# Goobley/Lightweaver

Measured on AMD Instinct MI355X. Metric: formal_sol_gamma_matrices iters/sec, higher is better.
Workload: dtype f64; 1 GPU; FALC 82-depth H(6)+CaII(6), 5 mu, Bezier3, densified wavelength grid; Nlambda_per_gpu=10240, Nlambda_total=10240, Nspace=82, Nrays=5, active_transitions=25, parallelism=single GPU, sweep=lanes

## Files before the change

include/lwhip.h:

```cpp
#ifndef LWHIP_H
#define LWHIP_H

#include <stddef.h>
#include <stdint.h>

#ifdef __cplusplus
extern "C" {
#endif

#define LWHIP_ABI_VERSION 4


enum { LWHIP_LINE = 0, LWHIP_CONTINUUM = 1 };

enum {
    LWHIP_BC_UNINITIALISED = 0,
    LWHIP_BC_ZERO = 1,
    LWHIP_BC_THERMALISED = 2,
    LWHIP_BC_PERIODIC = 3,
    LWHIP_BC_CALLABLE = 4
};

enum {
    LWHIP_FS_LINEAR_1D = 0,
// ... 347 lines not shown
    int32_t _pad;
    const double* muz;
    const double* vz;
    const double* lowerBc;
    double* I;
    double* depthChi;
    double* depthEta;
    double* depthI;
} lwhip_rays;
int lwhip_compute_rays(lwhip_context* ctx, const lwhip_rays* rays);
int lwhip_batch_compute_rays(lwhip_batch* batch, const lwhip_rays* perColumn);

int lwhip_synchronize(lwhip_context* ctx);

int lwhip_set_zplane_outputs(lwhip_context* ctx, double* zPlaneDown, double* zPlaneUp);

int lwhip_set_stream(lwhip_context* ctx, void* stream);

int lwhip_profile_enable(lwhip_context* ctx, int enable);
int lwhip_sweep_time(lwhip_context* ctx, double* meanMs, int* nLaunches);

int lwhip_algorithmic_bytes(lwhip_context* ctx, double* bytes);
int lwhip_sweep_kind(lwhip_context* ctx);

#ifdef __cplusplus
}
#endif
#endif
```

lightweaver_amd/_abi.py:

```python
import ctypes as C

ABI_VERSION = 4
AXIS_NONE, AXIS_X, AXIS_Z = 0, 1, 2

LINE, CONTINUUM = 0, 1
BC_UNINITIALISED, BC_ZERO, BC_THERMALISED, BC_PERIODIC, BC_CALLABLE = range(5)
FS_LINEAR_1D, FS_BESSER_1D, FS_BEZIER3_1D = range(3)
FS_NAMES = {
    'piecewise_linear_1d': FS_LINEAR_1D,
    'piecewise_besser_1d': FS_BESSER_1D,
    'piecewise_bezier3_1d': FS_BEZIER3_1D,
}
OK, ERR_INVALID, ERR_UNSUPPORTED, ERR_DEVICE, ERR_SINGULAR, ERR_BUSY = range(6)

ATMOS = 1 << 0
BACKGROUND = 1 << 1
PROFILES = 1 << 2
POPS = 1 << 3
NSTAR = 1 << 4
J = 1 << 5
GAMMA = 1 << 6
BC = 1 << 7
RHOPRD = 1 << 8
I = 1 << 9
# ... 197 lines not shown
    ('lwhip_batch_stat_equil', C.c_int, [C.c_void_p]),
    ('lwhip_batch_compute_profiles', C.c_int, [C.c_void_p]),
    ('lwhip_build_intersections', C.c_int, [C.POINTER(lwhip_grid2d), C.POINTER(lwhip_intersection),
                                             C.POINTER(lwhip_intersection), i32p, i32p, C.c_int32,
                                             C.POINTER(lwhip_intersection), C.c_int64, C.POINTER(C.c_int32),
                                             C.POINTER(C.c_int64)]),
    ('lwhip_redistribute_prd', C.c_int, [ctx_p, C.c_int, C.c_double, C.POINTER(lwhip_prd_result)]),
    ('lwhip_prd_pack', C.c_int, [ctx_p, C.POINTER(C.c_void_p), C.POINTER(C.c_size_t)]),
    ('lwhip_prd_partial', C.c_int, [ctx_p]),
    ('lwhip_prd_finalise', C.c_int, [ctx_p, f64p, i32p, f64p, i32p]),
    ('lwhip_ng_configure', C.c_int, [ctx_p, C.c_int, C.c_int, C.c_int]),
    ('lwhip_ng_accelerate', C.c_int, [ctx_p, i32p, f64p, i32p]),
    ('lwhip_time_dep_update', C.c_int, [ctx_p, C.c_int, f64p, C.c_double]),
    ('lwhip_nr_post_update', C.c_int, [ctx_p, C.POINTER(lwhip_nr_args)]),
    ('lwhip_set_depth_range', C.c_int, [ctx_p, C.c_int, C.c_int]),
    ('lwhip_set_djmax_index_mode', C.c_int, [ctx_p, C.c_int]),
    ('lwhip_synchronize', C.c_int, [ctx_p]),
    ('lwhip_set_stream', C.c_int, [ctx_p, C.c_void_p]),
    ('lwhip_set_zplane_outputs', C.c_int, [ctx_p, f64p, f64p]),
    ('lwhip_profile_enable', C.c_int, [ctx_p, C.c_int]),
    ('lwhip_sweep_time', C.c_int, [ctx_p, C.POINTER(C.c_double), C.POINTER(C.c_int)]),
    ('lwhip_algorithmic_bytes', C.c_int, [ctx_p, C.POINTER(C.c_double)]),
    ('lwhip_sweep_kind', C.c_int, [ctx_p]),
    ('lwhip_set_stokes', C.c_int, [ctx_p, C.POINTER(lwhip_stokes)]),
    ('lwhip_compute_polarised_profiles', C.c_int, [ctx_p]),
    ('lwhip_full_stokes_fs', C.c_int, [ctx_p, C.c_int, C.c_int, C.POINTER(lwhip_iter_result)]),
    ('lwhip_batch_compute_polarised_profiles', C.c_int, [C.c_void_p]),
    ('lwhip_batch_full_stokes_fs', C.c_int, [C.c_void_p, C.c_int, C.c_int, C.POINTER(lwhip_iter_result)]),
    ('lwhip_compute_rays', C.c_int, [ctx_p, C.POINTER(lwhip_rays)]),
    ('lwhip_batch_compute_rays', C.c_int, [C.c_void_p, C.POINTER(lwhip_rays)]),
]


def bind(lib):
    for name, restype, argtypes in SYMBOLS:
        fn = getattr(lib, name)
        fn.restype = restype
        fn.argtypes = argtypes
    return lib


def make_nr_args(atomIdxs, stages, backgroundNe, ne, dC=None, nPrev=None, dt=0.0, crsw=1.0):
    import numpy as np
    n = len(atomIdxs)
    idx = np.ascontiguousarray(atomIdxs, dtype=np.int32)

# ... 15 lines not shown
```

lightweaver_amd/context.py:

```python
from __future__ import annotations

import ctypes as C
import os
from dataclasses import dataclass
from typing import Optional

import numpy as np

from . import _abi as abi
from .model import Problem, check_mus

_PKG = os.path.dirname(os.path.abspath(__file__))
LIB_PATH = os.environ.get('LWHIP_LIB') or os.path.join(_PKG, 'liblwhip.so')
_lib = None


class LwHipError(RuntimeError):
    pass


class ExplodingMatrixError(Exception):
    """Singular Gamma in stat_equil (lightweaver.utils.ExplodingMatrixError)."""


# ... 437 lines not shown
            return False
        _check(self.lib, st, 'lwhip_map_host_J')
        return bool(enable)

    def fingerprint_J(self, array=None) -> int:
        import numpy as np
        ptr = (array if array is not None else self.prob.J[self.laStart:self.laEnd]).ctypes.data
        out = C.c_uint64()
        _check(self.lib, self.lib.lwhip_fingerprint_J(self._h, C.c_void_p(ptr), C.byref(out)), 'lwhip_fingerprint_J')
        return out.value

    def profile_enable(self, enable=True):
        _check(self.lib, self.lib.lwhip_profile_enable(self._h, int(enable)), 'lwhip_profile_enable')

    def sweep_time(self):
        ms = C.c_double()
        n = C.c_int()
        _check(self.lib, self.lib.lwhip_sweep_time(self._h, C.byref(ms), C.byref(n)), 'lwhip_sweep_time')
        return ms.value, n.value

    def sweep_kind(self):
        return {0: 'march', 1: 'lanes', 2: '2d'}.get(self.lib.lwhip_sweep_kind(self._h), '?')

    def algorithmic_bytes(self):
        b = C.c_double()
        _check(self.lib, self.lib.lwhip_algorithmic_bytes(self._h, C.byref(b)), 'lwhip_algorithmic_bytes')
        return b.value


def host_fingerprint(array) -> int:
    import numpy as np
    assert array.dtype == np.float64 and array.flags.c_contiguous
    return load_library().lwhip_host_fingerprint(array.ctypes.data_as(abi.f64p), array.size)


def device_count():
    return load_library().lwhip_device_count()
```

lightweaver_amd/csrc/lwhip_api.hip:

```cpp
#include "lwhip_host.h"

namespace
{
thread_local std::string g_lastError;
}

namespace lwhip
{
int fail(int code, const std::string& msg)
{
    g_lastError = msg;
    return code;
}
}

namespace
{
constexpr size_t HB_TAIL = 0, HB_STATUS = 32, HB_ZERO = 40, HB_POPSTATUS = 48, HB_TURNLATE = 56, HB_PRDCTL = 64, HB_CANARY = 96, HB_CHANGE = 128;
constexpr uint64_t HB_CANARY_WORD = 0x6c77686970424c4bull;
constexpr unsigned char HB_DEAD = 0xC5;
struct Quarantine
{
    std::mutex m;
    std::vector<std::pair<unsigned char*, size_t>> blocks;
// ... 702 lines not shown
    DevArena arena;
    H2DBatch h2d;
    auto bail = [&](int code) {
        h2d.close();
        if (c->tablesFrom)
            c->tablesFrom->borrowers--;
        delete c;
        return code;
    };
    if (hipSetDevice(c->device) != hipSuccess)
        return bail(fail(LWHIP_ERR_DEVICE, "hipSetDevice failed"));
    if (opts && opts->stream)
        c->stream = (hipStream_t)opts->stream;
    else
    {
        c->ownStreamShared = like != nullptr && c->batchHint > 1;
        if ((c->ownStreamShared ? stream_acquire_shared(c->device, &c->ownStream) : stream_acquire(c->device, &c->ownStream)) != hipSuccess)
            return bail(fail(LWHIP_ERR_DEVICE, "hipStreamCreate failed"));
        c->stream = c->ownStream;
    }
    if (host_block_init(c) != LWHIP_OK)
        return bail(LWHIP_ERR_DEVICE);
    c->pairRays = dbg_env_int("LWHIP_PAIR_RAYS", 1) != 0;
    c->prdPipeline = dbg_env_int("LWHIP_PRD_PIPELINE", 1) != 0;
    c->prdGeneral = dbg_env_int("LWHIP_PRD_GENERAL", 0) != 0;
    const bool timing = std::getenv("LWHIP_CREATE_TIMING") != nullptr;
    auto now = [] { return std::chrono::steady_clock::now(); };
    auto ms = [](auto a, auto b) { return std::chrono::duration<double, std::milli>(b - a).count(); };
    const auto t0 = now();
    c->structSig = structure_signature(c);
    if (like)
    {
        lwhip_context* owner = like->tablesFrom ? like->tablesFrom : like;
        if (owner->structSig != c->structSig)
            return bail(fail(LWHIP_ERR_INVALID, "lwhip_create_like: the problems differ in structure (sizes, solver, shard, wavelength "
                                                "grid, or a transition's levels / range / coefficients / grid / cross-sections)"));
        c->tablesFrom = owner;
    }
    const bool plainAllocs = poison_on() || sentinel_on() || std::getenv("LWHIP_TRACE_ALLOC") != nullptr;
    if (!plainAllocs)
    {
        if (c->tablesFrom && c->tablesFrom->stateBytes > 0)
        {
            arena.size = c->tablesFrom->stateBytes + (64u << 10);
            if (hipMalloc((void**)&arena.base, arena.size) == hipSuccess && hipMemsetAsync(arena.base, 0, arena.size, c->stream) == hipSuccess)
                c->stateArena = arena.base;
// ... 1064 lines not shown

int lwhip_sweep_time(lwhip_context* c, double* meanMs, int* nLaunches)
{
    if (!c)
        return fail(LWHIP_ERR_INVALID, "null context");
    HIP_TRY(hipSetDevice(c->device));
    int st = collect_profile(c);
    if (st != LWHIP_OK)
        return st;
    if (meanMs)
        *meanMs = c->sweepCount ? c->sweepMs / c->sweepCount : 0.0;
    if (nLaunches)
        *nLaunches = c->sweepCount;
    return LWHIP_OK;
}

int lwhip_sweep_kind(lwhip_context* c)
{
    if (!c)
        return -1;
    return c->is2d ? 2 : c->laneSweep ? 1 : 0;
}

int lwhip_algorithmic_bytes(lwhip_context* c, double* bytes)
{
    if (!c || !bytes)
        return fail(LWHIP_ERR_INVALID, "null argument");
    const double Ns = c->Ns, Nla = c->Nla, Nmu = c->Nrays;
    double sumLineLa = 0.0, gam = 0.0, lev = 0.0;
    for (auto& h : c->trans)
        if (h.t.type == LWHIP_LINE)
            sumLineLa += h.NredLoc - h.NblueLoc;
    for (auto& a : c->atoms)
    {
        lev += a.Nlevel;
        if (!a.detailed)
            gam += 2.0 * a.Nlevel * a.Nlevel;
    }
    double b = 8.0 * Ns * (2.0 * Nmu * sumLineLa + 3.0 * Nla + 2.0 * Nla);
    b += 8.0 * Nla * Nmu * c->Nx;
    b += 8.0 * Ns * (gam + lev);
    b += 8.0 * Ns * 2.0 * c->Ntrans;
    b += 8.0 * Ns * (lev + 3.0 + Nmu);
    *bytes = b;
    return LWHIP_OK;
}
// ... 2 lines not shown
```

lightweaver_amd/csrc/lwhip_batch.hip:

```cpp
#include "lwhip_host.h"


static int batch_compute_profiles(lwhip_batch* b, bool all)
{
    std::vector<VoigtLineArgs> list;
    std::vector<lwhip_context*> todo;
    for (lwhip_context* c : b->ctxs)
    {
        if (!(all || c->profilesStale))
            continue;
        const int st = voigt_line_list(c, list);
        if (st != LWHIP_OK)
            return st;
        todo.push_back(c);
    }
    if (todo.empty())
        return LWHIP_OK;
    lwhip_context* c0 = b->ctxs[0];
    if (!list.empty())
    {
        if (b->voigtList.n < list.size())
        {
            HIP_TRY(hipStreamSynchronize(c0->stream));
            HIP_TRY(b->voigtList.alloc(c0->mem, list.size()));
// ... 184 lines not shown
        if (stp != LWHIP_OK)
            return stp;
    }
    for (int i = 0; i < n; ++i)
    {
        lwhip_context* c = b->ctxs[i];
        if (c->partialPending || c->prdPending)
            return fail(LWHIP_ERR_INVALID, "batch iteration while a split iteration of a column is pending");
        c->prefillCrsw = crsw;
        c->dJPrdClean = false;
        c->prefillPending = c->gammaTot > 0 && c->Cmat.p != nullptr;
        b->aHost[i] = make_apply_args(c);
        c->prefillPending = false;
    }
    if (!b->aValid || b->aCrsw != crsw)
    {
        HIP_TRY(hipMemcpyAsync(b->aList.p, b->aHost.data(), (size_t)n * sizeof(ApplyArgs), hipMemcpyHostToDevice, c0->stream));
        b->aValid = true;
        b->aCrsw = crsw;
    }
    TileDyn dyn = make_dyn(c0, false, lambdaIterate);
    for (int q = 0; q < n && dyn.phiSym; ++q)
        dyn.phiSym = b->ctxs[q]->phiSym ? 1 : 0;
    const bool fuse = c0->tileFuse;
    if (!c0->laneSweep)
        HIP_TRY(launch_tile_pre(c0->dtargs.p, c0->htargs, c0->nTiles, b->apList.p, n, c0->stream));
    if (c0->laneSweep)
        HIP_TRY(launch_lane_sweep(c0->dtargs.p, c0->htargs, dyn, c0->prob.formalSolver, true, c0->nTileChunks, c0->tileWaves, b->apList.p, n,
                                  c0->stream));
    else
    {
        HIP_TRY(launch_tile_sweep(c0->dtargs.p, c0->htargs, dyn, c0->prob.formalSolver, c0->tileCap, true, fuse, c0->nTileChunks,
                                  c0->tileWaves, b->apList.p, n, c0->stream));
        if (!fuse)
            HIP_TRY(launch_tile_post(c0->dtargs.p, c0->htargs, dyn, c0->nPostChunks, b->apList.p, n, c0->stream));
    }
    {
        ReduceArgs r0 = make_reduce_args(c0);
        r0.zeroParts = 1;
        HIP_TRY(launch_reduce_sum(r0, c0->stream, b->rList.p, n));
    }
    if (c0->Natom > 0)
        HIP_TRY(launch_apply(b->aHost[0], c0->stream, b->aList.p, n));
    if (results)
    {
        HIP_TRY(hipMemcpyAsync(b->tailPinned.host, b->tail.p, (size_t)2 * n * sizeof(double), hipMemcpyDeviceToHost, c0->stream));
        HIP_TRY(hipStreamSynchronize(c0->stream));
        for (int i = 0; i < n; ++i)
        {
            results[i].updatedJ = 1;
            results[i].dJMax = b->tailPinned.as<double>()[2 * i];
            results[i].dJMaxIdx = (int32_t)b->tailPinned.as<double>()[2 * i + 1];
// ... 40 lines not shown
```

lightweaver_amd/csrc/lwhip_host.h:

```cpp
#pragma once
#include "lwhip_internal.h"
#include "../../include/lwhip.h"

#include <hip/hip_runtime.h>

#include <algorithm>
#include <array>
#include <atomic>
#include <cmath>
#include <cstdio>
#include <cstdlib>
#include <chrono>
#include <cstring>
#include <functional>
#include <map>
#include <memory>
#include <mutex>
#include <string>
#include <type_traits>
#include <vector>

namespace lwhip
{
int fail(int code, const std::string& msg);
// ... 367 lines not shown
    bool prdPending = false;
    bool prdFused = false;
    std::vector<std::unique_ptr<DevBuf<double>>> gII;
    std::vector<char> gIIValid;
    DevBuf<NrAtom> nrAtoms, statEqAtoms;
    DevBuf<NgAtom> ngAtoms;
    DevBuf<double> ngHistory;
    std::vector<NgAtom> ngAtomsHost;
    int ngOrder = 0, ngPeriod = 0, ngDelay = 0, ngCount = 0;
    bool ngConfigured = false;
    int statEqKey = -2;
    int32_t* statusHost = nullptr;
    int32_t* statusDev = nullptr;
    double* changeHost = nullptr;
    double* changeDev = nullptr;
    size_t changeCount = 0;
    DevBuf<int32_t> transType;
    DevBuf<int32_t> contLa;
    DevBuf<int32_t> prdChangeIdx;
    PinnedBlock prdPinned;
    DevBuf<int32_t> prdCtl;
    bool phiSym = false, vlosZero = false;
    bool pairRays = true, prdPipeline = true, prdGeneral = false;
    PinnedBlock prdPinnedPipe;
    int prdPipeIter = 0;
    double prdPipeTol = 0.0;
    DevBuf<DevTrans> dtrans;
    DevBuf<DevLaHeader> laHdr;
    DevBuf<DevSlot> slots;
    DevBuf<DevProgram> progs;
    DevBuf<DevProgRow> progRows;
    DevBuf<DevProgEnt> progEnts;
    DevBuf<ContArgs> dargs;
    ContArgs hargs{};
    bool atomicParts = false;
    bool red8Clean = false;
    int* zeroCheck = nullptr;
    int* zeroCheckDev = nullptr;
    DevBuf<int32_t> atomTrOffD, atomNlevel, atomDetailed, transLi, transLj;
    DevBuf<int64_t> atomGammaOff;
    DevBuf<double> red, red8, dJ;
    std::vector<double> gatherHost;
    DevBuf<int32_t> status;
    StokesState stokes;
    RaysState* rays = nullptr;

// ... 140 lines not shown
```

lightweaver_amd/csrc/lwhip_internal.h:

```cpp
#pragma once
#include <vector>
#include <hip/hip_runtime.h>
#include <stdint.h>

#include "../../include/lwhip.h"

namespace lwhip
{
constexpr double CLight = 2.99792458E+08;
constexpr double HPlanck = 6.6260755E-34;
constexpr double HC = HPlanck * CLight;
constexpr double KBoltzmann = 1.380658E-23;
constexpr double Pi = 3.14159265358979323846264338327950288;
constexpr double NM_TO_M = 1.0E-09;
constexpr double HC_K = HC / (KBoltzmann * NM_TO_M);
constexpr double HC_4PI = 0.25 * HC / Pi;
constexpr double PI4_HC = 1.0 / HC_4PI;
constexpr double PI4_H = 4.0 * Pi / HPlanck;
constexpr double TWO_HC_NM3 = 2.0 * HC / (NM_TO_M * NM_TO_M * NM_TO_M);

struct DevTrans
{
    int32_t type;
    int32_t atom;
// ... 230 lines not shown
    const int64_t* hJOff;
    const lwhip_j_coeff* hJCoef;
    double* JRest;
    const DevLaneWg* laneWg;
    const DevLaneTile* laneTiles;
    const DevLaneRay* laneRays;
    const DevLaneFin* laneFin;
    const double* laneFinPar;
    const double* bcPlanck;
    const uint8_t* laneFeedG;
    double* momS;
    int32_t momA, _padM;
    int32_t* turnLate;
    double* detSlab;
    double* lsDbg;
};
struct TileDyn
{
    int32_t nPass;
    int32_t lambdaIterate;
    int32_t prdOnly;
    int32_t stopIter;
    const int32_t* stopCtl;
    int32_t phiSym, _padS;
};
struct RetileArgs
{
    int32_t Ns, Nmu, L, nTiles;
    const DevTile* tiles;
    const DevTileSlot* tslots;
    const DevTrans* trans;
    const double* phi;
    double* phiT;
};
size_t raymarch_lds_bytes(const TileArgs& a, int waves, bool fuse);
hipError_t launch_tile_pre(const TileArgs* devArgs, const TileArgs& hostArgs, int nTilesLaunch, const TileArgs* const* apList,
                           int nBatch, hipStream_t stream);
hipError_t launch_tile_sweep(const TileArgs* devArgs, const TileArgs& hostArgs, const TileDyn& dyn, int solver, int cap,
                             bool rates, bool fuse, int nChunks, int waves, const TileArgs* const* apList, int nBatch,
                             hipStream_t stream);
hipError_t launch_tile_post(const TileArgs* devArgs, const TileArgs& hostArgs, const TileDyn& dyn, int nPostChunks,
                            const TileArgs* const* apList, int nBatch, hipStream_t stream);
bool lane_sweep_supported(int Ns, int Nrays, int solver, int* D, int* LR, int* R);
size_t lane_sweep_lds_bytes(const TileArgs& a, int waves);
hipError_t launch_lane_sweep(const TileArgs* devArgs, const TileArgs& hostArgs, const TileDyn& dyn, int solver, bool rates,
                             int nChunks, int waves, const TileArgs* const* apList, int nBatch, hipStream_t stream);
void dbg_scratch_poison(hipStream_t stream);
hipError_t launch_det_reduce(const double* slab, const int32_t* off, const int32_t* ent, double* part, int Ns, int Ntrans,
                             hipStream_t stream);
size_t det_reduce_scratch_doubles(int Ns, int Ntrans);
hipError_t launch_retile(const RetileArgs& a, hipStream_t stream);
hipError_t launch_retile_list(const RetileArgs* devList, const RetileArgs* hostList, int n, hipStream_t stream);

#ifndef LWHIP_REDUCE_SPLIT_N
#define LWHIP_REDUCE_SPLIT_N 4
#endif
enum { LWHIP_REDUCE_SPLIT = LWHIP_REDUCE_SPLIT_N };
enum { LWHIP_DET_SEG = 32 };
struct ReduceArgs
{
    int32_t Ns, Ntrans;
    double* red8;
    double* red;
    const double* dJ;
    int32_t Nla, idxOffset, world, rank;
    double* batchTail;
    int32_t zeroParts;
// ... 312 lines not shown
```

lightweaver_amd/csrc/lwhip_lanesweep.hip:

```cpp
#include "lwhip_device.h"
#include <atomic>
#include <cstdlib>
#include "../../include/lwhip.h"

#include <algorithm>
#include <type_traits>

namespace lwhip
{
namespace
{
typedef unsigned int ls_u2 __attribute__((ext_vector_type(2)));
typedef unsigned int ls_u4 __attribute__((ext_vector_type(4)));

DEVINL __amdgpu_buffer_rsrc_t ls_rsrc(const void* p, unsigned long long bytes)
{
    const unsigned n = bytes > 0xfffffff0ull ? 0xfffffff0u : (unsigned)bytes;
    return __builtin_amdgcn_make_buffer_rsrc((void*)p, 0, (int)n, 0x00020000);
}
template <int N> DEVINL void ls_ld(__amdgpu_buffer_rsrc_t r, unsigned voff, unsigned soff, double (&x)[N])
{
#pragma unroll
    for (int q = 0; q + 1 < N; q += 2)
    {
// ... 31 lines not shown
    const int lo = __builtin_amdgcn_update_dpp(0, (int)(unsigned)vv, CTRL, 0xf, 0xf, true);
    const int hi = __builtin_amdgcn_update_dpp(0, (int)(unsigned)(vv >> 32), CTRL, 0xf, 0xf, true);
    return __longlong_as_double(((unsigned long long)(unsigned)hi << 32) | (unsigned)lo);
}
DEVINL double ls_bperm(double v, int srcLane)
{
    const unsigned long long vv = __double_as_longlong(v);
    const int lo = __builtin_amdgcn_ds_bpermute(srcLane << 2, (int)(unsigned)vv);
    const int hi = __builtin_amdgcn_ds_bpermute(srcLane << 2, (int)(unsigned)(vv >> 32));
    return __longlong_as_double(((unsigned long long)(unsigned)hi << 32) | (unsigned)lo);
}
template <bool UP> DEVINL void ls_scan(double& E, double& B, const int lane, const int LR)
{
#pragma unroll
    for (int s = 1; s < 64; s <<= 1)
    {
        if (s == 32 && LR <= 32)
            break;
        const int src = UP ? lane + s : lane - s;
        const double Ep = ls_bperm(E, src), Bp = ls_bperm(B, src);
        B = fma(E, Bp, B);
        E = E * Ep;
    }
}
DEVINL double ls_rcp(double x)
{
    double r = __builtin_amdgcn_rcp(x);
    const double e = fma(-x, r, 1.0);
    return fma(r, e, r);
}
enum { LS_EXP_TAB = 32 };
DEVINL void ls_exp_table_init(double* tab, int t)
{
    if (t < LS_EXP_TAB)
        tab[t] = exp2((double)t * (1.0 / LS_EXP_TAB));
}
DEVINL double ls_exp_neg(double x, const double* tab)
{
    double k0 = 46.166241308446828384, k1 = -2.16608493865351192653e-02, k2 = -5.96317165397058656257e-12;
    double c6 = 1.0 / 720.0, c5 = 1.0 / 120.0, c4 = 1.0 / 24.0, c3 = 1.0 / 6.0;
    asm volatile("" : "+s"(k0), "+s"(k1), "+s"(k2), "+s"(c6), "+s"(c5), "+s"(c4), "+s"(c3));
    const double n = rint(x * k0);
    double r = fma(n, k1, x);
    r = fma(n, k2, r);
    const int ni = (int)n;
    const double T = tab[ni & (LS_EXP_TAB - 1)];
// ... 745 lines not shown
            LS_T(tp2);
            LS_TACC(tmB, tp1, tp2);
#pragma unroll
            for (int i = 0; i < D; ++i)
            {
                const double Su = SRC(i - 1), S0 = S[i];
                const double xi = x[i];
                const double x2 = xi * xi, x3 = x2 * xi;
                const double exr = ls_exp_neg(-fmin(xi, 64.0), c.sExp);
                const double ex = (xi > 30.0) ? 0.0 : exr;
                const double r3 = (rx[i] * rx[i]) * rx[i];
                const bool small = xi < 5e-2;
                auto pick = [&](double g, double t) {
                    LS_KEEP(g);
                    LS_KEEP(t);
                    double r = small ? t : g;
                    LS_KEEP(r);
                    return r;
                };
                const double xq = 0.25 * xi, q = 0.05 * x2, t3 = x3 * (1.0 / 120.0);
                const double al = pick((6.0 - ex * (6.0 + 6.0 * xi + 3.0 * x2 + x3)) * r3, xq - 4.0 * q + 10.0 * t3);
                const double be = pick((6.0 * ex - 6.0 + 6.0 * xi - 3.0 * x2 + x3) * r3, xq - q + t3);
                const double ga = pick(3.0 * (2.0 * xi - 6.0 + ex * (6.0 + 4.0 * xi + x2)) * r3, xq - 3.0 * q + 6.0 * t3);
                const double de = pick(3.0 * (6.0 - 4.0 * xi + x2 - 2.0 * ex * (3.0 + xi)) * r3, xq - 2.0 * q + 3.0 * t3);
                const double edt = pick(ex, 1.0 - xi + 0.5 * x2 - 20.0 * t3);
                const double x_3 = xi * (1.0 / 3.0);
                const double dSu = i == 0 ? dSP : dS[i > 0 ? i - 1 : 0];
                const double Cuw = Su + x_3 * dSu;
                const double C0 = S0 - x_3 * dS[i];
                double e1 = edt, b1 = al * Su + be * S0 + ga * Cuw + de * C0, ps = be + de;
                LS_KEEP(b1);
                LS_KEEP(ps);
                if (__builtin_amdgcn_ballot_w64(is_last(i)) != 0)
                {
                    double w0 = 1.0 - exr, w1 = (1.0 - exr) - xi * exr;
                    if (xi < 5.0E-4)
                    {
                        w0 = xi * (1.0 - 0.5 * xi);
                        w1 = (xi * xi) * (0.5 - xi * (1.0 / 3.0));
                    }
                    else if (xi > 50.0)
                        w0 = w1 = 1.0;
                    const double rL = ls_rcp(xi);
                    const double dSL = (S0 - Su) * rL;
                    const bool lst = is_last(i);
                    e1 = lst ? 1.0 - w0 : e1;
                    b1 = lst ? w0 * S0 - w1 * dSL : b1;
                    ps = lst ? w0 - w1 * rL : ps;
// ... 467 lines not shown
            static_assert(D % 2 == 0, "the block's rate integrals are formed in halves");
            if (!MOM)
            {
                rates_half(std::integral_constant<int, 0>{});
                LS_PHASE();
                rates_half(std::integral_constant<int, D / 2>{});
            }
        }
        LS_PHASE();
        LS_T(tp5);
        LS_TACC(tmA, tp0, tp1);
        LS_TACC(tmS, tp3, tp4);
        LS_TACC(tmD, tp4, tp5);
#ifdef LS_TIMING
        tmC += tp3 - tp1 - (tmB - tmBprev);
        tmBprev = tmB;
#endif
#undef MI
#undef IV
#undef CHI
#undef SRC
    };

    const int nRun = NRUN;
    for (run = 0; run < nRun; ++run)
    {
    const bool pairMode = PAIRABLE && dyn.phiSym != 0 && dyn.nPass == 2 && q0 == 0 && q1 == 2 * Nmu;
    if (!pairMode)
        prefetch_first();
    if constexpr (CONT)
        cont_unit(0);
#ifdef LS_ABL_NO_RAYS
    if (dyn.nPass == 77)
#else
    if (dyn.nPass == 2)
#endif
    {
        if (pairMode)
        {
            if constexpr (PAIRABLE)
            {
                for (int mu = 0; mu < Nmu; ++mu)
                {
                    cont_unit(mu);
                    pass(std::false_type{}, std::true_type{}, mu, 0u);
                    pass(std::true_type{}, std::true_type{}, mu, 0u);
                }
            }
        }
        else
        {
            for (int mu = q0 >> 1; 2 * mu < q1; ++mu)
            {
                if (2 * mu >= q0)
                    pass(std::false_type{}, std::false_type{}, mu, (unsigned)(mu * 2 + 1) * Ns8);
                if (2 * mu + 1 < q1)
                    pass(std::true_type{}, std::false_type{}, mu, (unsigned)(mu * 2 + 2) * Ns8);
            }
        }
    }
    else
// ... 1676 lines not shown
    *LR = lr;
    *R = std::min(64 / lr, (int)LS_MAX_R);
    return true;
}

size_t det_reduce_scratch_doubles(int Ns, int Ntrans) { return (size_t)std::max(Ntrans, 1) * DET_SEG * 4 * Ns; }

hipError_t launch_det_reduce(const double* slab, const int32_t* off, const int32_t* ent, double* part, int Ns, int Ntrans,
                             hipStream_t stream)
{
    if (Ntrans <= 0)
        return hipSuccess;
    LWHIP_LAUNCH(det_reduce_kernel, dim3((4 * Ns + 255) / 256, Ntrans, DET_SEG), dim3(256), 0, stream, slab, off, ent, part, Ns);
    return hipGetLastError();
}

size_t lane_sweep_lds_bytes(const TileArgs& a, int waves)
{
    return sizeof(double) * ((size_t)a.maxCT * 4 * a.laneLRD + (size_t)waves * LS_MAX_R * 5 + LS_EXP_TAB + (size_t)waves * 3 * 64 * a.laneD
                             + (size_t)waves * std::min(a.maxC, (int)LWHIP_POST_MAXC) * a.L * 3)
           + a.depBytes + (a.detSlab ? ((size_t)a.maxCT * a.laneD * sizeof(int) + 7) / 8 * 8 : 0);
}

#ifndef LS_ISA_ONLY
hipError_t launch_lane_sweep(const TileArgs* devArgs, const TileArgs& a, const TileDyn& dyn, int solver, bool rates, int nChunks,
                             int waves, const TileArgs* const* apList, int nBatch, hipStream_t stream)
{
    if (nChunks <= 0)
        return hipSuccess;
    if (waves < 1 || waves > LS_MAX_WAVES || a.laneD != 4)
        return hipErrorInvalidValue;
    if (solver == LWHIP_FS_LINEAR_1D)
        return rates ? launch_ls_t<LWHIP_FS_LINEAR_1D, 4, 3>(devArgs, a, dyn, nChunks, waves, apList, nBatch, stream)
                     : launch_ls_t<LWHIP_FS_LINEAR_1D, 4, 2>(devArgs, a, dyn, nChunks, waves, apList, nBatch, stream);
    if (solver == LWHIP_FS_BESSER_1D)
        return rates ? launch_ls_t<LWHIP_FS_BESSER_1D, 4, 3>(devArgs, a, dyn, nChunks, waves, apList, nBatch, stream)
                     : launch_ls_t<LWHIP_FS_BESSER_1D, 4, 2>(devArgs, a, dyn, nChunks, waves, apList, nBatch, stream);
    if (solver != LWHIP_FS_BEZIER3_1D)
        return hipErrorInvalidValue;
    const bool hprd = a.hRho != nullptr || a.hJOff != nullptr;
    if (rates)
        return hprd ? launch_ls_t<LWHIP_FS_BEZIER3_1D, 4, 3>(devArgs, a, dyn, nChunks, waves, apList, nBatch, stream)
                    : launch_ls_t<LWHIP_FS_BEZIER3_1D, 4, 1>(devArgs, a, dyn, nChunks, waves, apList, nBatch, stream);
    return hprd ? launch_ls_t<LWHIP_FS_BEZIER3_1D, 4, 2>(devArgs, a, dyn, nChunks, waves, apList, nBatch, stream)
                : launch_ls_t<LWHIP_FS_BEZIER3_1D, 4, 0>(devArgs, a, dyn, nChunks, waves, apList, nBatch, stream);
}
// ... 3 lines not shown
```

lightweaver_amd/csrc/lwhip_state.hip:

```cpp
#include "lwhip_host.h"

namespace lwhip
{
bool poison_on()
{
    static const bool poison = debug_knobs_on() && std::getenv("LWHIP_POISON") != nullptr;
    return poison;
}
bool sentinel_on()
{
    static const bool on = debug_knobs_on() && std::getenv("LWHIP_PAD_SENTINEL") != nullptr && *std::getenv("LWHIP_PAD_SENTINEL");
    return on;
}
static bool sentinel_for(int seq)
{
    if (!sentinel_on())
        return false;
    static int lo = 0, hi = -1;
    static bool parsed = false;
    if (!parsed)
    {
        const char* v = std::getenv("LWHIP_PAD_SENTINEL");
        if (v[0] == 'a')
        {
// ... 455 lines not shown
    r.tslots = c->tslots.p;
    r.trans = c->dtrans.p;
    r.phi = c->phi.p;
    r.phiT = c->phiT.p;
    return true;
}

int retile_profiles(lwhip_context* c)
{
    RetileArgs r;
    if (retile_args(c, r))
        HIP_TRY(launch_retile(r, c->stream));
    return LWHIP_OK;
}

TileDyn make_dyn(lwhip_context* c, bool upOnly, int lambdaIterate)
{
    TileDyn d{};
    d.nPass = upOnly ? 1 : 2;
    d.lambdaIterate = lambdaIterate;
    d.stopIter = 0;
    d.stopCtl = nullptr;
    d.phiSym = (c && c->phiSym && c->pairRays) ? 1 : 0;
    return d;
}

hipError_t run_sweep(lwhip_context* c, const TileDyn& dyn, bool rates, hipEvent_t e0, hipEvent_t e1)
{
    TileDyn td = dyn;
    const bool tprd = dyn.prdOnly != 0;
    if (tprd && c->nTileChunksPrd == 0)
        return hipSuccess;
    if (!tprd)
        c->dJPrdClean = false;
    const TileArgs* da = tprd ? c->dtargsPrd.p : c->dtargs.p;
    const TileArgs& ha = tprd ? c->htargsPrd : c->htargs;
    const bool fuse = c->tileFuse && rates;
    if (rates && c->hprd && c->JRest.p)
    {
        hipError_t ez = hipMemsetAsync(c->JRest.p, 0, c->JRest.n * sizeof(double), c->stream);
        if (ez != hipSuccess)
            return ez;
    }
    if (rates && c->zeroCheckDev)
    {
        hipError_t ec = launch_check_zero(c->red8.p, c->red8.n, c->zeroCheckDev, c->stream);
        if (ec != hipSuccess)
            return ec;
    }
    hipError_t e = c->laneSweep ? hipSuccess : launch_tile_pre(da, ha, tprd ? c->nTilesPrd : c->nTiles, nullptr, 0, c->stream);
    if (e != hipSuccess)
        return e;
    if (e0)
        (void)hipEventRecord(e0, c->stream);
    if (c->laneSweep)
        e = launch_lane_sweep(da, ha, td, c->prob.formalSolver, rates, tprd ? c->nTileChunksPrd : c->nTileChunks, c->tileWaves, nullptr, 0,
                              c->stream);
    else
        e = launch_tile_sweep(da, ha, td, c->prob.formalSolver, c->tileCap, rates, fuse, tprd ? c->nTileChunksPrd : c->nTileChunks,
                              (fuse && ha.depthSplit > 1) ? 2 * ha.depthSplit : c->tileWaves, nullptr, 0, c->stream);
    if (e1)
        (void)hipEventRecord(e1, c->stream);
    if (e == hipSuccess && rates && c->laneSweep && c->deterministic)
        e = launch_det_reduce(c->detSlab.p, tprd ? c->detOffPrd.p : c->detOff.p, tprd ? c->detEntPrd.p : c->detEnt.p, c->detPart.p, c->Ns,
                              c->Ntrans, c->stream);
    if (e != hipSuccess || !rates || fuse || c->laneSweep)
        return e;
    return launch_tile_post(da, ha, td, tprd ? c->nPostChunksPrd : c->nPostChunks, nullptr, 0, c->stream);
}

int flush_prefill(lwhip_context* c)
{
    if (c->prefillPending && c->gammaTot > 0)
        HIP_TRY(launch_prefill(c->Gamma.p, c->Cmat.p, c->prefillCrsw, (size_t)c->gammaTot, c->stream));
    c->prefillPending = false;
    return LWHIP_OK;
}

int verify_zero_check(lwhip_context* c)
{
// ... 455 lines not shown
```

lightweaver_amd/csrc/lwhip_tables.hip:

```cpp
#include "lwhip_host.h"

namespace lwhip
{
int validate(const lwhip_problem* p, std::string& why)
{
    if (!p)
    {
        why = "null problem";
        return LWHIP_ERR_INVALID;
    }
    if (p->abiVersion != LWHIP_ABI_VERSION)
    {
        why = "ABI version mismatch";
        return LWHIP_ERR_INVALID;
    }
    if (p->Nspace < 3 || p->Nrays < 1 || p->Nlambda < 1 || p->Natom < 0)
    {
        why = "need Nspace >= 3, Nrays >= 1, Nlambda >= 1";
        return LWHIP_ERR_INVALID;
    }
    if (p->grid2d)
    {
        const lwhip_grid2d& g = *p->grid2d;
        if (g.Nx < 2 || g.Nz < 2 || g.Nx > 1024 || g.Nx * g.Nz != p->Nspace || g.Nrays != p->Nrays)
// ... 1451 lines not shown
            auto wg_records = [&](const std::vector<int32_t>& chTile, const std::vector<int32_t>* order, const std::vector<int32_t>* split,
                                  int launchSplit) {
                const int nch = (int)chTile.size() - 1;
                std::vector<DevLaneWg> w(std::max(nch, 1));
                for (int b = 0; b < nch; ++b)
                {
                    const int ch = order ? (*order)[b] : b;
                    const int S = split ? (*split)[ch] : launchSplit;
                    w[b] = DevLaneWg{ ch, S > 1 ? S : 1, chTile[ch], chTile[ch + 1] };
                }
                return w;
            };
            std::vector<int32_t> orderHost;
            if (c->chunkOrderOn)
            {
                orderHost.resize(c->chunkOrder.n);
                if (c->mem.batch)
                    HIP_TRY(c->mem.batch->flush());
                HIP_TRY(hipMemcpyAsync(orderHost.data(), c->chunkOrder.p, orderHost.size() * sizeof(int32_t), hipMemcpyDeviceToHost, c->stream));
                HIP_TRY(hipStreamSynchronize(c->stream));
            }
            auto wgs = wg_records(chunkTile, c->chunkOrderOn ? &orderHost : nullptr, c->chunkSplitOn ? &laneChunkSplit : nullptr, c->laneSplit);
            HIP_TRY(c->laneWg.upload_or_borrow(c->mem, wgs, like ? &like->laneWg : nullptr));
            std::vector<int32_t> genOf(std::max<size_t>(tiles.size(), 1), -1);
            std::vector<uint8_t> feedG;
            c->nGenTiles = 0;
            auto feed_byte = [&](const DevSlot& cs, const DevTileSlot& us, bool isThisMixed) -> uint8_t {
                uint32_t b = 0;
                if ((cs.flags & 1) && (us.flags & 1))
                {
                    b |= cs.atom == us.atom ? 1u : 0u;
                    b |= cs.gi == us.gi ? 2u : 0u;
                    b |= cs.gj == us.gi ? 4u : 0u;
                    b |= cs.gi == us.gj ? 8u : 0u;
                    b |= cs.gj == us.gj ? 16u : 0u;
                    b |= cs.gj == us.gi ? 32u : 0u;
                    b |= cs.gj == us.gj ? 64u : 0u;
                }
                if (isThisMixed)
                    b |= 128u;
                return (uint8_t)b;
            };
            for (size_t t = 0; t < tiles.size(); ++t)
            {
                const DevTile& td = tiles[t];
                const bool fastKind = (td.nLine == 0 && td.nMixed == 0) || (td.nLine == 1 && td.nMixed <= 1) || (td.nLine == 2 && td.nMixed == 0);
// ... 154 lines not shown
```

Before: 7712 iters/s.

## Share Bezier3 coefficients between paired up/down rays in lane sweep

Adds a pair_pass in the lane sweep that computes the Bezier3 interpolation coefficients once per depth interval and uses them for both the downward and upward ray of a given mu. The two direction scans then run together in one interleaved prefix scan. This removes duplicated exp and polynomial coefficient work for continuum tiles and phi-symmetric line tiles. It enables this by default through an env flag and adds a debug counter for how many tasks take the path. It also increases register pressure from holding both directions' arrays at once, and disables FMA contraction in two places to keep results matching.

```diff
diff --git a/include/lwhip.h b/include/lwhip.h
--- a/include/lwhip.h
+++ b/include/lwhip.h
@@ -393,6 +393,7 @@
 
 int lwhip_algorithmic_bytes(lwhip_context* ctx, double* bytes);
 int lwhip_sweep_kind(lwhip_context* ctx);
+long lwhip_debug_pair_coef_tasks(lwhip_context* ctx);
 
 #ifdef __cplusplus
 }
diff --git a/lightweaver_amd/_abi.py b/lightweaver_amd/_abi.py
--- a/lightweaver_amd/_abi.py
+++ b/lightweaver_amd/_abi.py
@@ -243,6 +243,7 @@
     ('lwhip_sweep_time', C.c_int, [ctx_p, C.POINTER(C.c_double), C.POINTER(C.c_int)]),
     ('lwhip_algorithmic_bytes', C.c_int, [ctx_p, C.POINTER(C.c_double)]),
     ('lwhip_sweep_kind', C.c_int, [ctx_p]),
+    ('lwhip_debug_pair_coef_tasks', C.c_long, [ctx_p]),
     ('lwhip_set_stokes', C.c_int, [ctx_p, C.POINTER(lwhip_stokes)]),
     ('lwhip_compute_polarised_profiles', C.c_int, [ctx_p]),
     ('lwhip_full_stokes_fs', C.c_int, [ctx_p, C.c_int, C.c_int, C.POINTER(lwhip_iter_result)]),
diff --git a/lightweaver_amd/context.py b/lightweaver_amd/context.py
--- a/lightweaver_amd/context.py
+++ b/lightweaver_amd/context.py
@@ -483,6 +483,9 @@
     def sweep_kind(self):
         return {0: 'march', 1: 'lanes', 2: '2d'}.get(self.lib.lwhip_sweep_kind(self._h), '?')
 
+    def pair_coef_tasks(self):
+        return int(self.lib.lwhip_debug_pair_coef_tasks(self._h))
+
     def algorithmic_bytes(self):
         b = C.c_double()
         _check(self.lib, self.lib.lwhip_algorithmic_bytes(self._h, C.byref(b)), 'lwhip_algorithmic_bytes')
diff --git a/lightweaver_amd/csrc/lwhip_api.hip b/lightweaver_amd/csrc/lwhip_api.hip
--- a/lightweaver_amd/csrc/lwhip_api.hip
+++ b/lightweaver_amd/csrc/lwhip_api.hip
@@ -748,6 +748,7 @@
     if (host_block_init(c) != LWHIP_OK)
         return bail(LWHIP_ERR_DEVICE);
     c->pairRays = dbg_env_int("LWHIP_PAIR_RAYS", 1) != 0;
+    c->pairCoefs = dbg_env_int("LWHIP_PAIR_COEFS", 1) != 0;
     c->prdPipeline = dbg_env_int("LWHIP_PRD_PIPELINE", 1) != 0;
     c->prdGeneral = dbg_env_int("LWHIP_PRD_GENERAL", 0) != 0;
     const bool timing = std::getenv("LWHIP_CREATE_TIMING") != nullptr;
@@ -1858,6 +1859,8 @@
     return c->is2d ? 2 : c->laneSweep ? 1 : 0;
 }
 
+long lwhip_debug_pair_coef_tasks(lwhip_context* c) { return c ? c->pairCoefTasks : 0; }
+
 int lwhip_algorithmic_bytes(lwhip_context* c, double* bytes)
 {
     if (!c || !bytes)
diff --git a/lightweaver_amd/csrc/lwhip_batch.hip b/lightweaver_amd/csrc/lwhip_batch.hip
--- a/lightweaver_amd/csrc/lwhip_batch.hip
+++ b/lightweaver_amd/csrc/lwhip_batch.hip
@@ -230,12 +230,19 @@
     TileDyn dyn = make_dyn(c0, false, lambdaIterate);
     for (int q = 0; q < n && dyn.phiSym; ++q)
         dyn.phiSym = b->ctxs[q]->phiSym ? 1 : 0;
+    for (int q = 0; q < n && dyn.pairCoefs; ++q)
+        dyn.pairCoefs = b->ctxs[q]->pairCoefs ? 1 : 0;
     const bool fuse = c0->tileFuse;
     if (!c0->laneSweep)
         HIP_TRY(launch_tile_pre(c0->dtargs.p, c0->htargs, c0->nTiles, b->apList.p, n, c0->stream));
     if (c0->laneSweep)
+    {
         HIP_TRY(launch_lane_sweep(c0->dtargs.p, c0->htargs, dyn, c0->prob.formalSolver, true, c0->nTileChunks, c0->tileWaves, b->apList.p, n,
                                   c0->stream));
+        for (int q = 0; q < n; ++q)
+            b->ctxs[q]->pairCoefTasks =
+                lane_sweep_pairs_coefs(c0->htargs, dyn, c0->prob.formalSolver) ? c0->pairTasksCont + (dyn.phiSym ? c0->pairTasksLine : 0) : 0;
+    }
     else
     {
         HIP_TRY(launch_tile_sweep(c0->dtargs.p, c0->htargs, dyn, c0->prob.formalSolver, c0->tileCap, true, fuse, c0->nTileChunks,
diff --git a/lightweaver_amd/csrc/lwhip_host.h b/lightweaver_amd/csrc/lwhip_host.h
--- a/lightweaver_amd/csrc/lwhip_host.h
+++ b/lightweaver_amd/csrc/lwhip_host.h
@@ -413,6 +413,9 @@
     DevBuf<int32_t> prdCtl;
     bool phiSym = false, vlosZero = false;
     bool pairRays = true, prdPipeline = true, prdGeneral = false;
+    bool pairCoefs = true;
+    long pairCoefTasks = 0;
+    long pairTasksCont = 0, pairTasksLine = 0;
     PinnedBlock prdPinnedPipe;
     int prdPipeIter = 0;
     double prdPipeTol = 0.0;
diff --git a/lightweaver_amd/csrc/lwhip_internal.h b/lightweaver_amd/csrc/lwhip_internal.h
--- a/lightweaver_amd/csrc/lwhip_internal.h
+++ b/lightweaver_amd/csrc/lwhip_internal.h
@@ -276,7 +276,8 @@
     int32_t prdOnly;
     int32_t stopIter;
     const int32_t* stopCtl;
-    int32_t phiSym, _padS;
+    int32_t phiSym;
+    int32_t pairCoefs;
 };
 struct RetileArgs
 {
@@ -297,6 +298,7 @@
                             const TileArgs* const* apList, int nBatch, hipStream_t stream);
 bool lane_sweep_supported(int Ns, int Nrays, int solver, int* D, int* LR, int* R);
 size_t lane_sweep_lds_bytes(const TileArgs& a, int waves);
+bool lane_sweep_pairs_coefs(const TileArgs& hostArgs, const TileDyn& dyn, int solver);
 hipError_t launch_lane_sweep(const TileArgs* devArgs, const TileArgs& hostArgs, const TileDyn& dyn, int solver, bool rates,
                              int nChunks, int waves, const TileArgs* const* apList, int nBatch, hipStream_t stream);
 void dbg_scratch_poison(hipStream_t stream);
diff --git a/lightweaver_amd/csrc/lwhip_lanesweep.hip b/lightweaver_amd/csrc/lwhip_lanesweep.hip
--- a/lightweaver_amd/csrc/lwhip_lanesweep.hip
+++ b/lightweaver_amd/csrc/lwhip_lanesweep.hip
@@ -77,6 +77,31 @@
         B = fma(E, Bp, B);
         E = E * Ep;
     }
+}
+DEVINL void ls_scan_pair(double& Ed, double& Bd, double& Eu, double& Bu, const int lane, const int LR)
+{
+#pragma unroll
+    for (int s = 1; s < 64; s <<= 1)
+    {
+        if (s == 32 && LR <= 32)
+            break;
+        const double Epd = ls_bperm(Ed, lane - s), Bpd = ls_bperm(Bd, lane - s);
+        const double Epu = ls_bperm(Eu, lane + s), Bpu = ls_bperm(Bu, lane + s);
+        Bd = fma(Ed, Bpd, Bd);
+        Ed = Ed * Epd;
+        Bu = fma(Eu, Bpu, Bu);
+        Eu = Eu * Epu;
+    }
+}
+DEVINL double ls_add_nc(double c, double x)
+{
+#pragma clang fp contract(off)
+    return c + x;
+}
+DEVINL double ls_sub_nc(double c, double x)
+{
+#pragma clang fp contract(off)
+    return c - x;
 }
 DEVINL double ls_rcp(double x)
 {
@@ -868,8 +893,8 @@
                 const double al = pick((6.0 - ex * (6.0 + 6.0 * xi + 3.0 * x2 + x3)) * r3, xq - 4.0 * q + 10.0 * t3);
                 const double be = pick((6.0 * ex - 6.0 + 6.0 * xi - 3.0 * x2 + x3) * r3, xq - q + t3);
                 const double ga = pick(3.0 * (2.0 * xi - 6.0 + ex * (6.0 + 4.0 * xi + x2)) * r3, xq - 3.0 * q + 6.0 * t3);
-                const double de = pick(3.0 * (6.0 - 4.0 * xi + x2 - 2.0 * ex * (3.0 + xi)) * r3, xq - 2.0 * q + 3.0 * t3);
-                const double edt = pick(ex, 1.0 - xi + 0.5 * x2 - 20.0 * t3);
+                const double de = pick(3.0 * (6.0 - 4.0 * xi + x2 - 2.0 * ex * ls_add_nc(3.0, xi)) * r3, xq - 2.0 * q + 3.0 * t3);
+                const double edt = pick(ex, ls_sub_nc(1.0, xi) + 0.5 * x2 - 20.0 * t3);
                 const double x_3 = xi * (1.0 / 3.0);
                 const double dSu = i == 0 ? dSP : dS[i > 0 ? i - 1 : 0];
                 const double Cuw = Su + x_3 * dSu;
@@ -1383,6 +1408,270 @@
 #undef SRC
     };
 
+#ifdef LS_NO_PAIR_COEFS
+    constexpr bool PAIRCOEF = false;
+#else
+    constexpr bool PAIRCOEF = CONT || PAIRABLE;
+#endif
+    auto pair_pass = [&](const int mu) {
+        LS_T(tp0);
+        const double muz = CTAB(double, a.muz)[mu];
+        const double zmu = CTAB(double, a.muz)[Nmu + mu];
+        const double hw = act ? 0.5 * CTAB(double, a.wmu)[mu] : 0.0;
+        int pBot = c.pBot, blk = c.blk, nV = c.nV;
+        LS_KEEPI(pBot);
+        LS_KEEPI(blk);
+        LS_KEEPI(nV);
+        auto dhK = [&](const int q) { return ((const double*)(sDep + c.vK + c.oG))[q]; };
+        if (storeDepth && act)
+        {
+            const size_t o = ((size_t)(la * Nmu + mu) * 2) * Ns + k0;
+#pragma unroll
+            for (int p = 0; p < D; ++p)
+                if (p < c.nV)
+                {
+                    double eC = (c.sRow3 + c.lane * D)[64 * D + p];
+                    if constexpr (PAIRABLE)
+                        eC = fma(cer[0][p], hPhi[p], eC);
+                    GD(a.depthChi)[o + p] = hChi[p];
+                    GD(a.depthEta)[o + p] = eC;
+                    GD(a.depthChi)[o + Ns + p] = hChi[p];
+                    GD(a.depthEta)[o + Ns + p] = eC;
+                }
+        }
+        LS_PHASE();
+        LS_T(tp1);
+        auto chi_at = [&](const int i) {
+            const double* r3 = c.sRow3 + c.lane * D;
+            asm volatile("" : "+v"(r3));
+            double cC = r3[i];
+            if constexpr (PAIRABLE)
+                cC = fma(cxr[0][i], hPhi[i], cC);
+            return cC;
+        };
+        auto chiK = [&](int i) {
+            return i < 0 ? ls_shift1<true>(chi_at(D - 1)) : i >= D ? ls_shift1<false>(chi_at(0)) : chi_at(i < 0 ? 0 : i >= D ? D - 1 : i);
+        };
+        auto srcK = [&](int i) { return i < 0 ? hSLo : i >= D ? hSHi : hS[i < 0 ? 0 : i >= D ? D - 1 : i]; };
+        auto dsK = [&](int i) { return i < 0 ? hDSLo : i >= D ? hDSHi : hDS[i < 0 ? 0 : i >= D ? D - 1 : i]; };
+        struct XCoef
+        {
+            double al, be, ga, de, edt, x_3;
+        };
+        auto x_coefs = [&](const double xi, const double rxi) -> XCoef {
+            const double x2 = xi * xi, x3 = x2 * xi;
+            const double exr = ls_exp_neg(-fmin(xi, 64.0), c.sExp);
+            const double ex = (xi > 30.0) ? 0.0 : exr;
+            const double r3 = (rxi * rxi) * rxi;
+            const bool small = xi < 5e-2;
+            auto pick = [&](double g, double t) {
+                LS_KEEP(g);
+                LS_KEEP(t);
+                double r = small ? t : g;
+                LS_KEEP(r);
+                return r;
+            };
+            const double xq = 0.25 * xi, q = 0.05 * x2, t3 = x3 * (1.0 / 120.0);
+            XCoef k;
+            k.al = pick((6.0 - ex * (6.0 + 6.0 * xi + 3.0 * x2 + x3)) * r3, xq - 4.0 * q + 10.0 * t3);
+            k.be = pick((6.0 * ex - 6.0 + 6.0 * xi - 3.0 * x2 + x3) * r3, xq - q + t3);
+            k.ga = pick(3.0 * (2.0 * xi - 6.0 + ex * (6.0 + 4.0 * xi + x2)) * r3, xq - 3.0 * q + 6.0 * t3);
+            k.de = pick(3.0 * (6.0 - 4.0 * xi + x2 - 2.0 * ex * ls_add_nc(3.0, xi)) * r3, xq - 2.0 * q + 3.0 * t3);
+            k.edt = pick(ex, ls_sub_nc(1.0, xi) + 0.5 * x2 - 20.0 * t3);
+            k.x_3 = xi * (1.0 / 3.0);
+            return k;
+        };
+        auto form_map = [&](auto upTag, const int p, const XCoef& k, double& eo, double& bo, double& po) {
+            constexpr bool UP = decltype(upTag)::value;
+            const int pu = UP ? p + 1 : p - 1, pd = UP ? p - 1 : p + 1;
+            const int bcType = UP ? a.lowerBc : a.upperBc;
+            auto is_first = [&]() { return UP ? p == pBot : (p == 0 && blk == 0); };
+            auto is_last = [&]() { return UP ? (p == 0 && blk == 0) : p == pBot; };
+            auto is_ok = [&]() { return p < nV; };
+            const double Su = srcK(pu), S0 = hS[p];
+            const double dSu = UP ? -(dsK(pu) * muz) : dsK(pu) * muz;
+            const double dS0 = UP ? -(hDS[p] * muz) : hDS[p] * muz;
+            const double Cuw = Su + k.x_3 * dSu;
+            const double C0 = S0 - k.x_3 * dS0;
+            double e1 = k.edt, b1 = k.al * Su + k.be * S0 + k.ga * Cuw + k.de * C0, ps = k.be + k.de;
+            LS_KEEP(b1);
+            LS_KEEP(ps);
+            if (__builtin_amdgcn_ballot_w64(is_last()) != 0)
+            {
+                const bool lst = is_last();
+                const double dtL = ((0.5 * zmu) * (chiK(p) + chiK(pu))) * dhK(UP ? p + 1 : p);
+                const double xi = lst ? dtL : 1.0;
+                const double exr = ls_exp_neg(-fmin(xi, 64.0), c.sExp);
+                double w0 = 1.0 - exr, w1 = (1.0 - exr) - xi * exr;
+                if (xi < 5.0E-4)
+                {
+                    w0 = xi * (1.0 - 0.5 * xi);
+                    w1 = (xi * xi) * (0.5 - xi * (1.0 / 3.0));
+                }
+                else if (xi > 50.0)
+                    w0 = w1 = 1.0;
+                const double rL = ls_rcp(xi);
+                const double dSL = (S0 - Su) * rL;
+                e1 = lst ? 1.0 - w0 : e1;
+                b1 = lst ? w0 * S0 - w1 * dSL : b1;
+                ps = lst ? w0 - w1 * rL : ps;
+            }
+            if (__builtin_amdgcn_ballot_w64(is_first()) != 0)
+            {
+                double Ib = 0.0;
+                if (bcType == LWHIP_BC_THERMALISED)
+                {
+                    const double dtb = ((0.5 * zmu) * (chiK(p) + chiK(pd))) * dhK(UP ? p : p + 1);
+                    const double rdtb = ls_rcp(dtb);
+                    const double* sb = c.sB + min(c.rRaw, LS_MAX_R - 1) * 4 + (UP ? 2 : 0);
+                    const double B0 = sb[0], B1 = sb[1];
+                    Ib = UP ? B1 - (B0 - B1) * rdtb : B0 - (B1 - B0) * rdtb;
+                }
+                else if (bcType == LWHIP_BC_CALLABLE)
+                {
+                    const int mi = UP ? CTAB(int32_t, a.lowerIdx)[mu * 2 + 1] : CTAB(int32_t, a.upperIdx)[mu * 2 + 0];
+                    if (mi >= 0)
+                        Ib = UP ? GCD(a.lowerBcData)[(size_t)la * a.lowerNmu + mi] : GCD(a.upperBcData)[(size_t)la * a.upperNmu + mi];
+                }
+                const bool fst = is_first();
+                e1 = fst ? 0.0 : e1;
+                b1 = fst ? Ib : b1;
+                ps = fst ? 0.0 : ps;
+            }
+            if (__builtin_amdgcn_ballot_w64(!is_ok()) != 0)
+            {
+                const bool okk = is_ok();
+                e1 = okk ? e1 : 1.0;
+                b1 = okk ? b1 : 0.0;
+                ps = okk ? ps : 0.0;
+            }
+            eo = e1;
+            bo = b1;
+            po = (ps * hRch[p]) * lamf;
+        };
+        double pD[D], pU[D];
+        auto psi_sums = [&](const int p) {
+            if constexpr (RATES)
+            {
+                const double wD = hw * pD[p], wU = hw * pU[p];
+                M1[p] += wD;
+                if constexpr (NL > 0)
+                {
+                    const double wb = wD * hPhi[p];
+                    mQ1[p] += wb;
+                    mQ2[p] = fma(wb, hPhi[p], mQ2[p]);
+                }
+                M1[p] += wU;
+                if constexpr (NL > 0)
+                {
+                    const double wb = wU * hPhi[p];
+                    mQ1[p] += wb;
+                    mQ2[p] = fma(wb, hPhi[p], mQ2[p]);
+                }
+            }
+        };
+        double eD[D], bD[D], eU[D], bU[D];
+        {
+            const XCoef k = x_coefs(hT[0] * zmu, hRT[0] * muz);
+            XCoef kN;
+            kN.al = ls_shift1<false>(k.al);
+            kN.be = ls_shift1<false>(k.be);
+            kN.ga = ls_shift1<false>(k.ga);
+            kN.de = ls_shift1<false>(k.de);
+            kN.edt = ls_shift1<false>(k.edt);
+            kN.x_3 = (hT[D] * zmu) * (1.0 / 3.0);
+            form_map(std::false_type{}, 0, k, eD[0], bD[0], pD[0]);
+            form_map(std::true_type{}, D - 1, kN, eU[D - 1], bU[D - 1], pU[D - 1]);
+            LS_PHASE();
+        }
+#pragma unroll
+        for (int q = 1; q < D; ++q)
+        {
+            const XCoef k = x_coefs(hT[q] * zmu, hRT[q] * muz);
+            form_map(std::false_type{}, q, k, eD[q], bD[q], pD[q]);
+            form_map(std::true_type{}, q - 1, k, eU[q - 1], bU[q - 1], pU[q - 1]);
+            psi_sums(q - 1);
+            if (q == D - 1)
+                psi_sums(D - 1);
+            LS_PHASE();
+        }
+        LS_T(tp3);
+
+        double Id, Iu;
+        {
+            double Ed = 1.0, Bd = 0.0, Eu = 1.0, Bu = 0.0;
+#pragma unroll
+            for (int i = 0; i < D; ++i)
+            {
+                Bd = fma(eD[i], Bd, bD[i]);
+                Ed = eD[i] * Ed;
+                Bu = fma(eU[D - 1 - i], Bu, bU[D - 1 - i]);
+                Eu = eU[D - 1 - i] * Eu;
+            }
+            ls_scan_pair(Ed, Bd, Eu, Bu, c.lane, LR);
+            Id = ls_shift1<true>(Bd);
+            Iu = ls_shift1<false>(Bu);
+        }
+        LS_PHASE();
+        LS_T(tp4);
+
+        auto ray_out = [&](auto upTag, const double(&ee)[D], const double(&bb)[D], double I) {
+            constexpr bool UP = decltype(upTag)::value;
+            double Iv[D];
+#pragma unroll
+            for (int i = 0; i < D; ++i)
+            {
+                I = fma(ee[UP ? D - 1 - i : i], I, bb[UP ? D - 1 - i : i]);
+                Iv[UP ? D - 1 - i : i] = I;
+            }
+            int la = c.la;
+            LS_KEEPI(la);
+            if (UP && act && c.blk == 0)
+                GD(a.I)[(size_t)la * Nmu + mu] = Iv[0];
+            if ((UP ? a.zUp : a.zDown) != nullptr && act)
+            {
+#pragma unroll
+                for (int p = 0; p < D; ++p)
+                    if (k0 + p == (UP ? 1 : Ns - 2))
+                        GD(UP ? a.zUp : a.zDown)[(size_t)la * Nmu + mu] = Iv[p];
+            }
+            if (storeDepth && act)
+            {
+                const size_t o = ((size_t)(la * Nmu + mu) * 2 + (UP ? 1 : 0)) * Ns + k0;
+#pragma unroll
+                for (int p = 0; p < D; ++p)
+                    if (p < nV)
+                        GD(a.depthI)[o + p] = Iv[p];
+            }
+            if (RATES)
+            {
+#pragma unroll
+                for (int p = 0; p < D; ++p)
+                    Jk[p] += hw * Iv[p];
+                mW += hw;
+                if constexpr (NL > 0)
+                {
+#pragma unroll
+                    for (int p = 0; p < D; ++p)
+                    {
+                        const double wa = hw * hPhi[p];
+                        mP0[p] += wa;
+                        mP1[p] = fma(wa, Iv[p], mP1[p]);
+                    }
+                }
+            }
+        };
+        ray_out(std::false_type{}, eD, bD, Id);
+        LS_PHASE();
+        ray_out(std::true_type{}, eU, bU, Iu);
+        LS_PHASE();
+        LS_T(tp5);
+        LS_TACC(tmA, tp0, tp1);
+        LS_TACC(tmC, tp1, tp3);
+        LS_TACC(tmS, tp3, tp4);
+        LS_TACC(tmD, tp4, tp5);
+    };
+
     const int nRun = NRUN;
     for (run = 0; run < nRun; ++run)
     {
@@ -1397,7 +1686,32 @@
     if (dyn.nPass == 2)
 #endif
     {
-        if (pairMode)
+        const bool pairCoefs = PAIRCOEF && dyn.pairCoefs != 0;
+        if (pairMode && pairCoefs)
+        {
+            if constexpr (PAIRABLE)
+            {
+                for (int mu = 0; mu < Nmu; ++mu)
+                {
+                    cont_unit(mu);
+                    pair_pass(mu);
+                }
+            }
+        }
+        else if (CONT && pairCoefs)
+        {
+            if constexpr (CONT)
+            {
+                const int muA = (q0 + 1) >> 1, muB = q1 >> 1;
+                if (q0 & 1)
+                    pass(std::true_type{}, std::false_type{}, q0 >> 1, 0u);
+                for (int mu = muA; mu < muB; ++mu)
+                    pair_pass(mu);
+                if (q1 & 1)
+                    pass(std::false_type{}, std::false_type{}, q1 >> 1, 0u);
+            }
+        }
+        else if (pairMode)
         {
             if constexpr (PAIRABLE)
             {
@@ -3120,6 +3434,16 @@
            + a.depBytes + (a.detSlab ? ((size_t)a.maxCT * a.laneD * sizeof(int) + 7) / 8 * 8 : 0);
 }
 
+bool lane_sweep_pairs_coefs(const TileArgs& a, const TileDyn& dyn, int solver)
+{
+#ifdef LS_NO_PAIR_COEFS
+    return false;
+#else
+    const bool hprd = a.hRho != nullptr || a.hJOff != nullptr;
+    return solver == LWHIP_FS_BEZIER3_1D && !hprd && dyn.nPass == 2 && dyn.pairCoefs != 0;
+#endif
+}
+
 #ifndef LS_ISA_ONLY
 hipError_t launch_lane_sweep(const TileArgs* devArgs, const TileArgs& a, const TileDyn& dyn, int solver, bool rates, int nChunks,
                              int waves, const TileArgs* const* apList, int nBatch, hipStream_t stream)
diff --git a/lightweaver_amd/csrc/lwhip_state.hip b/lightweaver_amd/csrc/lwhip_state.hip
--- a/lightweaver_amd/csrc/lwhip_state.hip
+++ b/lightweaver_amd/csrc/lwhip_state.hip
@@ -501,6 +501,7 @@
     d.stopIter = 0;
     d.stopCtl = nullptr;
     d.phiSym = (c && c->phiSym && c->pairRays) ? 1 : 0;
+    d.pairCoefs = (c && c->pairCoefs) ? 1 : 0;
     return d;
 }
 
@@ -533,8 +534,12 @@
     if (e0)
         (void)hipEventRecord(e0, c->stream);
     if (c->laneSweep)
+    {
         e = launch_lane_sweep(da, ha, td, c->prob.formalSolver, rates, tprd ? c->nTileChunksPrd : c->nTileChunks, c->tileWaves, nullptr, 0,
                               c->stream);
+        if (!tprd)
+            c->pairCoefTasks = lane_sweep_pairs_coefs(ha, td, c->prob.formalSolver) ? c->pairTasksCont + (td.phiSym ? c->pairTasksLine : 0) : 0;
+    }
     else
         e = launch_tile_sweep(da, ha, td, c->prob.formalSolver, c->tileCap, rates, fuse, tprd ? c->nTileChunksPrd : c->nTileChunks,
                               (fuse && ha.depthSplit > 1) ? 2 * ha.depthSplit : c->tileWaves, nullptr, 0, c->stream);
diff --git a/lightweaver_amd/csrc/lwhip_tables.hip b/lightweaver_amd/csrc/lwhip_tables.hip
--- a/lightweaver_amd/csrc/lwhip_tables.hip
+++ b/lightweaver_amd/csrc/lwhip_tables.hip
@@ -1497,6 +1497,23 @@
             }
             auto wgs = wg_records(chunkTile, c->chunkOrderOn ? &orderHost : nullptr, c->chunkSplitOn ? &laneChunkSplit : nullptr, c->laneSplit);
             HIP_TRY(c->laneWg.upload_or_borrow(c->mem, wgs, like ? &like->laneWg : nullptr));
+            c->pairTasksCont = c->pairTasksLine = 0;
+            for (const DevLaneWg& w : wgs)
+                for (int t = w.t0; t < w.t1 && t < (int)tiles.size(); ++t)
+                {
+                    const DevTile& td = tiles[t];
+                    if (td.nLine == 0 && td.nMixed == 0)
+                    {
+                        const int nRays = 2 * c->Nrays, sh = w.split == 4 ? 2 : w.split == 2 ? 1 : 0;
+                        for (int sub = 0; sub < w.split; ++sub)
+                        {
+                            const int q0 = (sub * nRays) >> sh, q1 = ((sub + 1) * nRays) >> sh;
+                            c->pairTasksCont += 2 * ((q0 + 1) >> 1) + 1 < q1 ? 1 : 0;
+                        }
+                    }
+                    else if (td.nLine == 1 && td.nMixed <= 1 && w.split == 1)
+                        c->pairTasksLine++;
+                }
             std::vector<int32_t> genOf(std::max<size_t>(tiles.size(), 1), -1);
             std::vector<uint8_t> feedG;
             c->nGenTiles = 0;
```

Result: no change. 7742 iters/s, median of 6 (+0.4%).
